# sisl/NeRFSafetyValidation

Hardware: AMD Instinct MI355X
Metric: rendered_samples_per_sec (higher is better)
Workload: dtype f16; 1 GPU; Stonehenge 800x800 synthetic, hashgrid L=16 F=2 T=2^19 + ffmlp(64,2)/(64,3), fp16, occupancy-grid ray marching (run_cuda eval path, BASELINE configs[1]); rays_per_frame=640000, bound=2, cascade=2, frames_in_flight=3, fused_reference_rounding=True, parallelism=single GPU, rccl_ranks=1

## Files before the change

### nerfsafetyvalidation_amd/csrc/fused_net.hpp

```cpp
#pragma once
#include <hip/hip_fp16.h>
#include <math.h>

#include "ngp_common.hpp"

namespace ngp {

typedef _Float16 half8 __attribute__((ext_vector_type(8)));
typedef _Float16 half2v __attribute__((ext_vector_type(2)));
typedef _Float16 half4 __attribute__((ext_vector_type(4)));
typedef float f32x4 __attribute__((ext_vector_type(4)));

struct LevelTab {
    float scale[16];
    uint32_t offset[16], size[16];
    uint32_t a1[16], a2[16];
    uint32_t mask[16];
    uint32_t flags[16];
    uint32_t cell_off[16], cell_res[16];
};

struct NetArgs {
    const uint32_t* table;
    const _Float16* packed;
// ... 859 lines not shown
struct DebugState {
    int flags = 0;
    unsigned long long* stamps = nullptr;
    uint32_t* sample_hash = nullptr;
    bool coarse_off() const { return (flags & 2) != 0; }
    bool sort_off() const { return (flags & 4) != 0; }
    bool lin_off() const { return (flags & 8) != 0; }
    bool jump_off() const { return (flags & 1) != 0; }
    bool spec_off() const { return (flags & 256) != 0; }
    bool tile_off() const { return (flags & 8192) != 0; }
    bool pre_verdict_off() const { return (flags & 16384) != 0; }
    bool narrow_items_off() const { return (flags & 32768) != 0; }
    bool prefix_replay_off() const { return (flags & 65536) != 0; }
    bool wave_march_off() const { return (flags & 131072) != 0; }
    bool cell_runs_off() const { return (flags & 262144) != 0; }
    uint32_t spec_safety_x2() const { return ((uint32_t)flags >> 9) & 15u; }
    uint32_t shrink() const { return ((uint32_t)flags >> 4) & 15u; }
};
DebugState debug_snapshot();
float* grad_dump();
bool needs_generic(const GridLevels& lv);
int fill_net(const ngp_model* m, const DebugState& dbg, const _Float16* packed, NetArgs& na, GridLevels& lv);
size_t weights_bytes(const NetArgs& na);
uint32_t resident_blocks(size_t lds);
int net_variant(const NetArgs& na, const GridLevels& lv);
bool bwd_shape_ok(const NetArgs& na);
#define NGP_WITH_NET(variant, ...)                                           \
    switch (variant) {                                                       \
        case 0: { using NET = NetF16<0>; __VA_ARGS__; } break;               \
        case 1: { using NET = NetF16<1>; __VA_ARGS__; } break;               \
// ... 10 lines not shown
```

### nerfsafetyvalidation_amd/csrc/render_fused.hip

```cpp
#include <hip/hip_fp16.h>
#include <math.h>
#include <string.h>

#include <atomic>

#include "fused_net.hpp"
#include "occupancy.hpp"

namespace ngp {

constexpr int kWaves = 8;
constexpr int kThreads = kWaves * 64;
constexpr int kWavesPerSimd = 4;
constexpr int kCh = 2;
constexpr int kSlots = 64 * kCh;
constexpr size_t kLinMaxBytes = 4u << 20;
constexpr int kLookahead = 4;
constexpr int kRing = 8;

struct Ctl {
    uint32_t n_alive, n_step, step, done;
    uint32_t iters, last_n_alive, last_n_step, pad;
    unsigned long long samples_marched, samples_slots;
    uint32_t spec, rollbacks, backoff, rsv;
// ... 14 lines not shown
    const float *rays_o, *rays_d, *fars;
    float* rays_t;
    float *weights_sum, *depth, *image;
    float *last_sigmas, *last_rgbs;
    float pad_sigma, pad_r, pad_g, pad_b;
    float4* dump_rec;
    uint32_t* dump_iter;
    const int32_t* alive_in;
    int32_t* staging;
    uint32_t* chunk_count;
    uint32_t sort_slow;
    Ctl* ctl;
    QueueHeads* heads;
    unsigned long long* stat_shards;
    uint32_t* death_shards;
    float4* backup;
    const uint8_t* bitfield;
    uint32_t cascade, grid_size, max_steps, perturb;
    float dt_gamma;
    Pcg32 rng;
    OccupancyLin occ;
    uint32_t block_jump;
    uint32_t* sample_hash;
    unsigned long long* stamps;
    float2* march_samples;
    uint8_t* march_counts;
    uint32_t wave_slots;
    uint32_t n_rays;
    uint32_t pre_verdict;
    uint32_t wave_march_max;
// ... 31 lines not shown
    uint16_t list[kSlots];
    float od[64][6];
};

__device__ __forceinline__ void dump_row(const RenderArgs& ra, uint32_t entry, int32_t ray, uint32_t n_step, uint32_t k, float sg, float r,
                                         float g, float b) {
    if (ra.dump_rec) {
        ra.dump_rec[(size_t)ray * 8 + k] = make_float4(sg, r, g, b);
    } else {
        const size_t row = (size_t)entry * n_step + k;
        ra.last_sigmas[row] = sg;
        ra.last_rgbs[row * 3] = r; ra.last_rgbs[row * 3 + 1] = g; ra.last_rgbs[row * 3 + 2] = b;
    }
}

__device__ __forceinline__ void march_ahead_wave(const RenderArgs& ra, float bound, const Ctl& ctl, const uint32_t* coarse) {
    const uint32_t lane = threadIdx.x & 63u;
    const uint32_t entry = blockIdx.x * 4u + (threadIdx.x >> 6);
    if (entry >= ctl.n_alive) return;
    const uint32_t n_step = ctl.n_step, spec = ctl.spec;
    const int32_t ray = ra.alive_in[entry];
    Dda dda;
    const float t_c = ra.rays_t[ray], far = ra.fars[ray];
    float t_march = dda.start(ra.rays_o + (size_t)ray * 3, ra.rays_d + (size_t)ray * 3, ra.bitfield, bound, 0.0f, ra.max_steps, ra.cascade,
                              ra.grid_size, &ra.occ, ra.block_jump != 0, t_c, ra.perturb, ra.rng, entry);
    float last_m = t_march, geo_tc = t_c;
    uint32_t emitted = 0, rounds = 0;
    float2* out = ra.march_samples + ((size_t)(entry >> 6) * n_step) * 64 + (entry & 63u);
    while (t_march < far && emitted < n_step) {
        rounds++;
        const LatticeWindow w = probe_window(dda, t_march, far, lane, coarse);
        const uint32_t room = spec ? spec - emitted % spec : n_step - emitted;
        unsigned long long emit = 0ull;
        uint32_t cur = 0, cnt = 0;
        float t_next = t_march;
        for (int guard = 0; guard < 64; guard++) {
// ... 19 lines not shown
    }
    if (lane != 0) return;
    if (ra.stamps) {
        atomicAdd(ra.stamps + 4, (unsigned long long)rounds);
        atomicAdd(ra.stamps + 5, (unsigned long long)rounds * 64ull);
        atomicAdd(ra.stamps + 6, 1ull);
        atomicMax(ra.stamps + 7, (unsigned long long)rounds);
    }
    if (spec && ra.pre_verdict && emitted < n_step)
        atomicAdd(ra.death_shards + (size_t)kDeathShards * kSpecK + (blockIdx.x % kDeathShards) * kSpecK + emitted / spec, 1u);
    bool slow = false;
    if (ra.sort_slow && emitted == n_step) slow = geo_tc < far && dda.coarse_empty_at_lin(geo_tc, coarse);
    ra.march_counts[entry] = (uint8_t)(emitted | (slow ? 128u : 0u));
}

template <bool LIN>
__global__ void __launch_bounds__(256) k_march_ahead(RenderArgs ra, float bound) {
    const Ctl ctl = *ra.ctl;
    if (ctl.done) return;
    const uint32_t n_alive = ctl.n_alive, n_step = ctl.n_step, spec = ctl.spec;
    const bool by_wave = LIN && n_alive <= ra.wave_march_max;
    if (blockIdx.x * (by_wave ? 4u : 256u) >= n_alive) return;
    __shared__ uint32_t coarse_lds[kCoarseMaxBytes / 4];
    stage_coarse(ra.occ, coarse_lds, blockDim.x);
    __syncthreads();
    const uint32_t* coarse = ra.occ.coarse_words ? coarse_lds : nullptr;
    if (LIN && by_wave) {
        march_ahead_wave(ra, bound, ctl, coarse);
        return;
    }
    const uint32_t entry = blockIdx.x * blockDim.x + threadIdx.x;
    if (entry >= n_alive) return;
    const int32_t ray = ra.alive_in[entry];
    Dda dda;
    const float t_c = ra.rays_t[ray], far = ra.fars[ray];
    float t_march = dda.start(ra.rays_o + (size_t)ray * 3, ra.rays_d + (size_t)ray * 3, ra.bitfield, bound, ra.dt_gamma, ra.max_steps, ra.cascade,
                              ra.grid_size, LIN ? &ra.occ : nullptr, ra.block_jump != 0, t_c, ra.perturb, ra.rng, entry);
    float last_m = t_march;
    float geo_tc = t_c;
    uint32_t emitted = 0;
    float2* out = ra.march_samples + ((size_t)(entry >> 6) * n_step) * 64 + (entry & 63u);
    float x, y, z, dt;
    uint32_t probes = 0, probes_coarse_empty = 0, probes_fine_empty = 0;
    const bool run_cells = LIN && dda.const_dt && ra.cell_runs != 0;
    float occ_until = 0.0f;
    while (t_march < far && emitted < n_step) {
        probes++;
        const bool diag_ce = LIN && ra.stamps && dda.coarse_empty_at_lin(t_march, coarse);
// ... 43 lines not shown
        uint32_t* ex = ra.death_shards + (size_t)kDeathShards * kSpecK + (blockIdx.x % kDeathShards) * kSpecK;
        for (uint32_t j = 0; j < K; j++) {
            const unsigned long long b = __ballot(jd == j);
            if (leader && b) atomicAdd(&ex[j], (uint32_t)__popcll(b));
        }
    }
    bool slow = false;
    if (ra.sort_slow && emitted == n_step) slow = geo_tc < far && (LIN ? dda.coarse_empty_at_lin(geo_tc, coarse) : dda.coarse_empty_at(geo_tc, coarse));
    ra.march_counts[entry] = (uint8_t)(emitted | (slow ? 128u : 0u));
}

template <int MODE, bool HACC = false>
__global__ void __launch_bounds__(kThreads, kWavesPerSimd) k_render_iter(NetArgs na, GridLevels lv, RenderArgs ra) {
    Ctl ctl = *ra.ctl;
    if (ctl.done) return;
    const uint32_t n_step_marched = ctl.n_step;
    extern __shared__ __attribute__((aligned(16))) char smem[];
    if (ctl.spec) {
        uint32_t* exhausted = reinterpret_cast<uint32_t*>(smem);
        if (threadIdx.x < kSpecK) {
            uint32_t d = 0;
            for (int sh = 0; sh < kDeathShards; sh++) d += ra.death_shards[(size_t)kDeathShards * kSpecK + sh * kSpecK + threadIdx.x];
            exhausted[threadIdx.x] = d;
        }
        __syncthreads();
        truncate_launch(ctl, exhausted, ra.n_rays);
        __syncthreads();
    }
    const uint32_t n_alive = ctl.n_alive, n_step = ctl.n_step;
    const uint32_t spec = ctl.spec;
// ... 240 lines not shown
        wave_total += wave_samples;
        if (ra.dump_iter && active) ra.dump_iter[ray] = ctl.iters;
        if (ra.last_sigmas && !ra.dump_rec && !spec && chunk == n_chunks - 1) {
            for (uint32_t i = lane; i < 128; i += 64) {
                const size_t row = (size_t)n_alive * n_step + i;
                ra.last_sigmas[row] = ra.pad_sigma;
                ra.last_rgbs[row * 3] = ra.pad_r; ra.last_rgbs[row * 3 + 1] = ra.pad_g; ra.last_rgbs[row * 3 + 2] = ra.pad_b;
            }
        }
        NGP_STAMP(3)
    }
#undef NGP_STAMP
    if (lane == 0 && wave_total) atomicAdd(&ra.stat_shards[(blockIdx.x * kWaves + wid) % kStatShards], wave_total);
}

__device__ __forceinline__ void publish_status(unsigned long long* host_slot, const Ctl& n, uint32_t seq, unsigned long long* fin = nullptr,
                                               uint32_t call_tag = 0) {
    if (!host_slot) return;
    if (n.done && fin) {
        const unsigned long long tag = (unsigned long long)(0x8000u | (call_tag & 0x7FFFu)) << 48;
        __hip_atomic_store(fin + 0, tag | (n.samples_marched & 0xFFFFFFFFFFFFull), __ATOMIC_RELAXED, __HIP_MEMORY_SCOPE_SYSTEM);
        __hip_atomic_store(fin + 1, tag | (n.samples_slots & 0xFFFFFFFFFFFFull), __ATOMIC_RELAXED, __HIP_MEMORY_SCOPE_SYSTEM);
        __hip_atomic_store(fin + 2, tag | ((unsigned long long)(n.iters & 0xFFFFFFu) << 24) | (n.rollbacks & 0xFFFFFFu), __ATOMIC_RELAXED,
                           __HIP_MEMORY_SCOPE_SYSTEM);
        __hip_atomic_store(fin + 3, tag | ((unsigned long long)n.last_n_alive << 8) | (n.last_n_step & 0xFFu), __ATOMIC_RELAXED,
                           __HIP_MEMORY_SCOPE_SYSTEM);
    }
    const unsigned long long w = ((unsigned long long)seq << 32) | ((unsigned long long)(n.done ? 1u : 0u) << 31) | (n.n_alive & 0x7FFFFFFFu);
    __hip_atomic_store(host_slot, w, __ATOMIC_RELAXED, __HIP_MEMORY_SCOPE_SYSTEM);
}

__global__ void __launch_bounds__(256) k_render_compact(const Ctl* __restrict__ cur, Ctl* __restrict__ nxt, const int32_t* __restrict__ staging,
                                                         const uint32_t* __restrict__ chunk_count, int32_t* __restrict__ alive_out, uint32_t N,
                                                         uint32_t max_steps, const unsigned long long* __restrict__ stat_shards,
                                                         QueueHeads* __restrict__ nxt_heads, unsigned long long* __restrict__ host_slot, uint32_t seq,
                                                         const uint32_t* __restrict__ death_shards, uint32_t spec_allowed, const int32_t* __restrict__ alive_in,
                                                         const float4* __restrict__ backup, float* __restrict__ rays_t, float* __restrict__ weights_sum,
                                                         float* __restrict__ depth, float* __restrict__ image, uint32_t* __restrict__ sample_hash,
                                                         unsigned long long* stat_shards_rw, uint32_t* __restrict__ death_next, uint32_t wave_slots,
                                                         uint32_t cap_mid_max, uint32_t cap_hi, unsigned long long* __restrict__ fin_host, uint32_t call_tag) {
    __shared__ uint32_t red[3][4];
    __shared__ uint32_t off_f[9], off_s[9];
    Ctl c = *cur;
    if (c.done) {
        if (blockIdx.x == 0 && threadIdx.x == 0) {
            *nxt = c;
            publish_status(host_slot, c, seq, fin_host, call_tag);
        }
        return;
    }
    const uint32_t W = item_width(c.n_alive, wave_slots);
    const uint32_t n_chunks = (c.n_alive + W - 1) / W;
    const uint32_t n_blocks = (n_chunks + 7) / 8;
    const uint32_t g = blockIdx.x;
    if (g >= n_blocks) return;
    const uint32_t first = g * 8;
    __shared__ uint32_t deaths[kSpecK], exhausted[kSpecK];
    __shared__ uint32_t verdict_bad, verdict_keep;
    if (threadIdx.x < kSpecK) {
        uint32_t d = 0, x = 0;
        if (c.spec)
            for (int sh = 0; sh < kDeathShards; sh++) {
                d += death_shards[sh * kSpecK + threadIdx.x];
                x += death_shards[(size_t)kDeathShards * kSpecK + sh * kSpecK + threadIdx.x];
            }
        deaths[threadIdx.x] = d;
        exhausted[threadIdx.x] = x;
    }
    __syncthreads();
    truncate_launch(c, exhausted, N);
    if (threadIdx.x == 0) {
        uint32_t bad = 0, keep = 0;
        if (c.spec) {
            const uint32_t q = c.spec, K = c.n_step / q;
            uint32_t alive = c.n_alive;
            keep = K;
            for (uint32_t j = 0; j < K; j++) {
                if (alive == 0) break;
                const uint32_t want_q = N / alive;
                if (j > 0 && (want_q < 1 ? 1u : (want_q > 8 ? 8u : want_q)) != q) { bad = 1; keep = j; break; }
                alive -= deaths[j];
                if ((spec_allowed & 2u) && alive == 0) { bad = 1; keep = j; break; }
            }
        }
        verdict_bad = bad;
        verdict_keep = keep;
    }
    __syncthreads();
    if (verdict_bad) {
        for (uint32_t e = first * W + threadIdx.x; e < (first + 8) * W && e < c.n_alive; e += 256) {
            const int32_t ray = alive_in[e];
            const float4 a = backup[(size_t)ray * 2], b = backup[(size_t)ray * 2 + 1];
            rays_t[ray] = a.x; weights_sum[ray] = a.y; depth[ray] = a.z;
            if (sample_hash) sample_hash[ray] = __float_as_uint(a.w);
            image[(size_t)ray * 3] = b.x; image[(size_t)ray * 3 + 1] = b.y; image[(size_t)ray * 3 + 2] = b.z;
            alive_out[e] = ray;
        }
        if (g == n_blocks - 1 && threadIdx.x == 0) {
            Ctl n = c;
            n.rollbacks = c.rollbacks + 1;
            if (verdict_keep >= 2 && !(spec_allowed & 4u)) {
                n.spec = c.spec;
                n.n_step = verdict_keep * c.spec;
                n.backoff = 0;
                for (uint32_t i = 0; i < kDeathWords; i++) death_next[i] = 0;
            } else {
                n.spec = 0;
                const uint32_t ns = c.n_alive ? N / c.n_alive : 8;
                n.n_step = ns < 1 ? 1 : (ns > 8 ? 8 : ns);
                n.backoff = 2;
            }
            for (int i = 0; i < kStatShards; i++) stat_shards_rw[i] = 0ull;
            *nxt = n;
            for (int i = 0; i < 8; i++) nxt_heads->head[i][0] = 0;
            publish_status(host_slot, n, seq, fin_host, call_tag);
        }
        return;
    }
    uint32_t pf = 0, ps = 0, tf = 0;
    for (uint32_t j = threadIdx.x; j < n_chunks; j += 256) {
        const uint32_t v = chunk_count[j];
        tf += v >> 16;
        if (j < first) { pf += v & 0xffffu; ps += v >> 16; }
    }
#pragma unroll
    for (int off = 32; off > 0; off >>= 1) {
        pf += __shfl_down(pf, off, 64);
        ps += __shfl_down(ps, off, 64);
        tf += __shfl_down(tf, off, 64);
    }
    if ((threadIdx.x & 63) == 0) { red[0][threadIdx.x >> 6] = pf; red[1][threadIdx.x >> 6] = ps; red[2][threadIdx.x >> 6] = tf; }
    if (threadIdx.x == 0) {
        uint32_t af = 0, as = 0;
        for (uint32_t i = 0; i < 8; i++) {
            const uint32_t v = (first + i < n_chunks) ? chunk_count[first + i] : 0;
            off_f[i] = af; off_s[i] = as;
            af += v & 0xffffu; as += v >> 16;
        }
        off_f[8] = af; off_s[8] = as;
    }
    __syncthreads();
    const uint32_t prefix_f = red[0][0] + red[0][1] + red[0][2] + red[0][3];
    const uint32_t prefix_s = red[1][0] + red[1][1] + red[1][2] + red[1][3];
    const uint32_t total_s = red[2][0] + red[2][1] + red[2][2] + red[2][3];
    const uint32_t lane = threadIdx.x & 63, w = threadIdx.x >> 6;
#pragma unroll
    for (uint32_t h = 0; h < 2; h++) {
        const uint32_t ci = w * 2 + h;
        const uint32_t nf = off_f[ci + 1] - off_f[ci], ns = off_s[ci + 1] - off_s[ci];
        if (lane < ns) alive_out[prefix_s + off_s[ci] + lane] = staging[(size_t)(first + ci) * W + W - 1 - lane];
        if (lane < nf) alive_out[total_s + prefix_f + off_f[ci] + lane] = staging[(size_t)(first + ci) * W + lane];
    }
    unsigned long long marched = threadIdx.x < (uint32_t)kStatShards ? stat_shards_rw[threadIdx.x] : 0ull;
#pragma unroll
    for (int off = 32; off > 0; off >>= 1) marched += __shfl_down(marched, off, 64);
    if (g == n_blocks - 1 && threadIdx.x == 0) {
        Ctl n = c;
        n.samples_marched = c.samples_marched + marched;
        for (int i = 0; i < kStatShards; i++) stat_shards_rw[i] = 0ull;
        n.n_alive = total_s + prefix_f + off_f[8];
        uint32_t recent = c.n_alive - n.n_alive;
        if (!c.spec) {
            n.last_n_alive = c.n_alive;
            n.last_n_step = c.n_step;
            n.iters = c.iters + 1;
            n.samples_slots = c.samples_slots + (unsigned long long)c.n_alive * c.n_step;
            n.step = c.step + c.n_step;
        } else {
            const uint32_t q = c.spec, K = c.n_step / q;
            uint32_t alive = c.n_alive, d_last = 0, d_prev = 0;
            unsigned long long slots = c.samples_slots;
            uint32_t it = 0;
            for (uint32_t j = 0; j < K; j++) {
                if (alive == 0) break;
                slots += (unsigned long long)alive * q;
                it++;
                n.last_n_alive = alive;
                n.last_n_step = q;
                alive -= deaths[j];
                d_prev = d_last;
                d_last = deaths[j];
            }
            recent = d_last > d_prev ? d_last : d_prev;
            n.iters = c.iters + it;
            n.samples_slots = slots;
            n.step = c.step + it * q;
        }
        uint32_t ns = n.n_alive ? N / n.n_alive : 8;
        n.n_step = ns < 1 ? 1 : (ns > 8 ? 8 : ns);
        n.done = (n.n_alive == 0 || n.step >= max_steps) ? 1 : 0;
        n.spec = 0;
        if (n.backoff) n.backoff--;
        else if (spec_allowed && !n.done && n.n_step <= kSpecMaxQ && (n.n_step == 8 || n.n_alive > N / (n.n_step + 1))) {
            const uint32_t q = n.n_step;
            const bool own_last = (spec_allowed & 2u) != 0;
            uint32_t room = (max_steps - n.step) / q;
            if (own_last && room) room--;
            const uint32_t headroom = n.n_alive - (q == 8 ? 0u : N / (q + 1)) - 1;
            uint32_t sq = 0;
            while ((unsigned long long)(sq + 1) * (sq + 1) <= recent) sq++;
            const unsigned long long rate = (unsigned long long)recent + 4ull * sq + 16ull;
            const uint32_t safety_x2 = (spec_allowed >> 8) ? (spec_allowed >> 8) : kSpecSafetyX2;
            uint32_t K = (uint32_t)((unsigned long long)headroom * 2u / (safety_x2 * rate));
            const uint32_t cap_mid = 8u * q < cap_mid_max ? 8u * q : cap_mid_max;
            const uint32_t cap_samples = q == 1 ? 8u : (q <= 4 ? cap_mid : cap_hi);
            const uint32_t capK = cap_samples / q < kSpecK ? cap_samples / q : kSpecK;
            K = (q == 8 && !own_last) ? capK : (K < capK ? K : capK);
            K = K < room ? K : room;
            if (K >= 2) { n.spec = q; n.n_step = K * q; }
        }
        if (n.spec)
            for (uint32_t i = 0; i < kDeathWords; i++) death_next[i] = 0;
        *nxt = n;
        for (int i = 0; i < 8; i++) nxt_heads->head[i][0] = 0;
        publish_status(host_slot, n, seq, fin_host, call_tag);
    }
}

__global__ void __launch_bounds__(256) k_render_init(uint32_t N, const float* __restrict__ nears, float* __restrict__ rays_t,
                                                      int32_t* __restrict__ alive, float* __restrict__ weights_sum, float* __restrict__ depth,
                                                      float* __restrict__ image, Ctl* __restrict__ ctl, uint32_t max_steps,
                                                      uint32_t* __restrict__ sample_hash, unsigned long long* __restrict__ stat_shards,
                                                      QueueHeads* __restrict__ heads, uint32_t* __restrict__ death_shards, uint32_t spec_allowed,
                                                      uint32_t tile_w) {
    const uint32_t n = blockIdx.x * 256 + threadIdx.x;
    if (n < (uint32_t)kStatShards) stat_shards[n] = 0ull;
    if (n < 2u * kDeathWords) death_shards[n] = 0;
    if (n < 16) heads[n >> 3].head[n & 7][0] = 0;
    if (n < N) {
        if (sample_hash) sample_hash[n] = 2166136261u;
// ... 299 lines not shown
    uint32_t known = 0;
    uint32_t launches = 2;
    bool done = false;
    while (!done) {
        const uint32_t cur = launched & 1;
        const uint32_t chunks = items_bound(ub, ra.wave_slots);
        static const uint32_t pct_env = getenv("NGP_ITER_BLOCKS_PCT") ? (uint32_t)atoi(getenv("NGP_ITER_BLOCKS_PCT")) : 0u;
        const uint32_t blocks_pct = pct_env ? pct_env : (g_active_renders.load(std::memory_order_relaxed) > 1 ? 62u : 100u);
        const uint32_t max_blocks = (uint32_t)ctx->num_cu * blocks_per_cu * blocks_pct / 100u;
        const uint32_t want_blocks = div_up(chunks, kWaves);
        const uint32_t blocks = want_blocks < max_blocks ? want_blocks : max_blocks;
        ra.alive_in = ctx->alive[cur];
        ra.ctl = ctx->ctl + cur;
        ra.heads = ctx->heads + cur;
        ra.death_shards = ctx->death_shards + (size_t)cur * kDeathWords;
        {
            ProfScope pm("k_march_ahead", s, 0);
            const uint32_t by_wave = div_up(ub < ra.wave_march_max ? ub : ra.wave_march_max, 4);
            const uint32_t by_lane = div_up(ub ? ub : 1, 256);
            if (lin) k_march_ahead<true><<<by_lane > by_wave ? by_lane : by_wave, 256, 0, s>>>(ra, na.bound);
            else k_march_ahead<false><<<div_up(ub ? ub : 1, 256), 256, 0, s>>>(ra, na.bound);
        }
        {
            ProfScope pk("k_render_iter", s, 0);
            iter_kernel<<<blocks, kThreads, lds, s>>>(na, lv, ra);
        }
        k_render_compact<<<div_up(chunks, 8), 256, 0, s>>>(ctx->ctl + cur, ctx->ctl + (cur ^ 1), ctx->staging, ctx->chunk_count,
                                                           ctx->alive[cur ^ 1], N, max_steps, ctx->stat_shards, ctx->heads + (cur ^ 1),
                                                           ctx->status_dev + launched % kRing, ctx->seq_base + launched + 1,
                                                           ctx->death_shards + (size_t)cur * kDeathWords, spec_allowed, ctx->alive[cur],
                                                           ctx->backup, ctx->rays_t, weights_sum, depth, image, dbg.sample_hash, ctx->stat_shards,
                                                           ctx->death_shards + (size_t)(cur ^ 1) * kDeathWords, ra.wave_slots, cap_mid_max, cap_hi, ctx->fin_dev, call_tag);
        launched++;
        launches += 3;
        while (known < launched) {
            static const uint32_t lookahead = getenv("NGP_LOOKAHEAD") ? (uint32_t)atoi(getenv("NGP_LOOKAHEAD")) : (uint32_t)kLookahead;
            const bool must_wait = launched - known >= lookahead;
            volatile unsigned long long* slot = ctx->status + known % kRing;
            const uint32_t want_seq = ctx->seq_base + known + 1;
            unsigned long long w = *slot;
            if ((uint32_t)(w >> 32) != want_seq) {
                if (!must_wait) break;
                uint32_t spins = 0;
                while ((uint32_t)((w = *slot) >> 32) != want_seq) {
                    if ((++spins & 0xFFFFFu) == 0) {
                        const hipError_t q = hipStreamQuery(s);
                        if (q != hipSuccess && q != hipErrorNotReady) {
                            set_error("render_rays: %s", hipGetErrorString(q));
                            return NGP_ELAUNCH;
                        }
                        if (q == hipSuccess && (uint32_t)(*slot >> 32) != want_seq) {
// ... 6 lines not shown
            }
            known++;
            ub = (uint32_t)w & 0x7FFFFFFFu;
            static const bool trace_sched = getenv("NGP_TRACE_SCHEDULE") != nullptr;
            if (trace_sched) fprintf(stderr, "[ngp] call %u launch %u: n_alive %u%s\n", call_tag, known, ub, ((w >> 31) & 1ull) ? " done" : "");
            if ((w >> 31) & 1ull) { done = true; break; }
        }
        if (launched > 2u * max_steps + 16u) {
            set_error("render_rays: iteration bound exceeded");
            return NGP_ELAUNCH;
        }
    }
    ctx->seq_base += launched;
    if (ra.dump_rec) {
        const uint32_t nb = div_up(N, 256);
        const Ctl* fin_state = ctx->ctl + (launched & 1);
        k_dump_count<<<nb, 256, 0, s>>>(ctx->dump_iter, N, fin_state, ctx->chunk_count);
        k_dump_scan<<<1, 1024, 0, s>>>(ctx->chunk_count, nb);
        k_dump_gather<<<nb, 256, 0, s>>>(ctx->dump_iter, ctx->dump_rec, N, fin_state, ctx->chunk_count,
                                         last_sigmas, last_rgbs, ra.pad_sigma, ra.pad_r, ra.pad_g, ra.pad_b);
    }
    rc = check_launch("render_rays");
    if (rc) return rc;
    bool have_fin = false;
    Ctl fin = {};
    if (stats_host && !sync) {
        volatile unsigned long long* f = ctx->fin;
        unsigned long long w[4] = {0, 0, 0, 0};
        for (uint32_t spin = 0; spin < 200000u && !have_fin; spin++) {
            bool all = true;
            for (int i = 0; i < 4; i++) {
// ... 5 lines not shown
        }
        if (have_fin) {
            fin.samples_marched = w[0] & 0xFFFFFFFFFFFFull;
            fin.samples_slots = w[1] & 0xFFFFFFFFFFFFull;
            fin.iters = (uint32_t)((w[2] >> 24) & 0xFFFFFFu);
            fin.rollbacks = (uint32_t)(w[2] & 0xFFFFFFu);
            fin.last_n_alive = (uint32_t)((w[3] >> 8) & 0xFFFFFFFFu);
            fin.last_n_step = (uint32_t)(w[3] & 0xFFu);
        }
    }
    if ((stats_host && !have_fin) || sync) {
        if (hipStreamSynchronize(s) != hipSuccess) {
            set_error("render_rays: %s", hipGetErrorString(hipGetLastError()));
            return NGP_ELAUNCH;
        }
        if (hipMemcpy(&fin, ctx->ctl + (launched & 1), sizeof(Ctl), hipMemcpyDeviceToHost) != hipSuccess) {
            set_error("render_rays: %s", hipGetErrorString(hipGetLastError()));
            return NGP_ELAUNCH;
        }
        have_fin = true;
    }
    if (have_fin) {
        if (stats_host) {
            stats_host->samples_marched = fin.samples_marched;
            stats_host->samples_slots = fin.samples_slots;
            stats_host->iterations = fin.iters;
            stats_host->rays = N;
            stats_host->last_n_alive = fin.last_n_alive;
            stats_host->last_n_step = fin.last_n_step;
            stats_host->launches = launches;
            stats_host->replayed = fin.rollbacks;
// ... 17 lines not shown
```

Baseline: 7.704 billion samples/s.

## Fuse compaction and control-state update into the next march kernel

The per-iteration compaction kernel is removed as a separate launch. Each march block now recomputes the launch verdict and next control state, and gathers its own slice of surviving rays directly from chunk counts and staging before marching. This cuts one kernel launch per iteration and the round trip through the alive list, but every block redundantly reads the death shards and chunk-count prefix. The host scheduling loop is adjusted because the status for an iteration is now published one launch later.

Result: slower. 7.561 billion samples/s (-1.9%).

```diff
diff --git a/nerfsafetyvalidation_amd/csrc/fused_net.hpp b/nerfsafetyvalidation_amd/csrc/fused_net.hpp
--- a/nerfsafetyvalidation_amd/csrc/fused_net.hpp
+++ b/nerfsafetyvalidation_amd/csrc/fused_net.hpp
@@ -897,6 +897,7 @@
     bool prefix_replay_off() const { return (flags & 65536) != 0; }
     bool wave_march_off() const { return (flags & 131072) != 0; }
     bool cell_runs_off() const { return (flags & 262144) != 0; }
+    bool fused_stitch_off() const { return (flags & 524288) != 0; }
     uint32_t spec_safety_x2() const { return ((uint32_t)flags >> 9) & 15u; }
     uint32_t shrink() const { return ((uint32_t)flags >> 4) & 15u; }
 };
diff --git a/nerfsafetyvalidation_amd/csrc/render_fused.hip b/nerfsafetyvalidation_amd/csrc/render_fused.hip
--- a/nerfsafetyvalidation_amd/csrc/render_fused.hip
+++ b/nerfsafetyvalidation_amd/csrc/render_fused.hip
@@ -52,6 +52,7 @@
     QueueHeads* heads;
     unsigned long long* stat_shards;
     uint32_t* death_shards;
+    uint32_t* death_next;
     float4* backup;
     const uint8_t* bitfield;
     uint32_t cascade, grid_size, max_steps, perturb;
@@ -113,12 +114,285 @@
     }
 }
 
-__device__ __forceinline__ void march_ahead_wave(const RenderArgs& ra, float bound, const Ctl& ctl, const uint32_t* coarse) {
+__device__ __forceinline__ void publish_status(unsigned long long* host_slot, const Ctl& n, uint32_t seq, unsigned long long* fin = nullptr,
+                                               uint32_t call_tag = 0) {
+    if (!host_slot) return;
+    if (n.done && fin) {
+        const unsigned long long tag = (unsigned long long)(0x8000u | (call_tag & 0x7FFFu)) << 48;
+        __hip_atomic_store(fin + 0, tag | (n.samples_marched & 0xFFFFFFFFFFFFull), __ATOMIC_RELAXED, __HIP_MEMORY_SCOPE_SYSTEM);
+        __hip_atomic_store(fin + 1, tag | (n.samples_slots & 0xFFFFFFFFFFFFull), __ATOMIC_RELAXED, __HIP_MEMORY_SCOPE_SYSTEM);
+        __hip_atomic_store(fin + 2, tag | ((unsigned long long)(n.iters & 0xFFFFFFu) << 24) | (n.rollbacks & 0xFFFFFFu), __ATOMIC_RELAXED,
+                           __HIP_MEMORY_SCOPE_SYSTEM);
+        __hip_atomic_store(fin + 3, tag | ((unsigned long long)n.last_n_alive << 8) | (n.last_n_step & 0xFFu), __ATOMIC_RELAXED,
+                           __HIP_MEMORY_SCOPE_SYSTEM);
+    }
+    const unsigned long long w = ((unsigned long long)seq << 32) | ((unsigned long long)(n.done ? 1u : 0u) << 31) | (n.n_alive & 0x7FFFFFFFu);
+    __hip_atomic_store(host_slot, w, __ATOMIC_RELAXED, __HIP_MEMORY_SCOPE_SYSTEM);
+}
+
+__device__ __forceinline__ void load_launch_counts(const Ctl& c, const uint32_t* __restrict__ death_shards, uint32_t* deaths, uint32_t* exhausted) {
+    if (threadIdx.x < kSpecK) {
+        uint32_t d = 0, x = 0;
+        if (c.spec)
+            for (int sh = 0; sh < kDeathShards; sh++) {
+                d += death_shards[sh * kSpecK + threadIdx.x];
+                x += death_shards[(size_t)kDeathShards * kSpecK + sh * kSpecK + threadIdx.x];
+            }
+        deaths[threadIdx.x] = d;
+        exhausted[threadIdx.x] = x;
+    }
+}
+__device__ __forceinline__ bool launch_verdict(const Ctl& c, const uint32_t* deaths, uint32_t N, uint32_t spec_allowed, uint32_t& keep) {
+    keep = 0;
+    if (!c.spec) return false;
+    const uint32_t q = c.spec, K = c.n_step / q;
+    uint32_t alive = c.n_alive;
+    keep = K;
+    for (uint32_t j = 0; j < K; j++) {
+        if (alive == 0) break;
+        const uint32_t want_q = N / alive;
+        if (j > 0 && (want_q < 1 ? 1u : (want_q > 8 ? 8u : want_q)) != q) { keep = j; return true; }
+        alive -= deaths[j];
+        if ((spec_allowed & 2u) && alive == 0) { keep = j; return true; }
+    }
+    return false;
+}
+__device__ __forceinline__ Ctl rollback_ctl(const Ctl& c, uint32_t keep, uint32_t N, uint32_t spec_allowed) {
+    Ctl n = c;
+    n.rollbacks = c.rollbacks + 1;
+    if (keep >= 2 && !(spec_allowed & 4u)) {
+        n.spec = c.spec;
+        n.n_step = keep * c.spec;
+        n.backoff = 0;
+    } else {
+        n.spec = 0;
+        const uint32_t ns = c.n_alive ? N / c.n_alive : 8;
+        n.n_step = ns < 1 ? 1 : (ns > 8 ? 8 : ns);
+        n.backoff = 2;
+    }
+    return n;
+}
+__device__ __forceinline__ Ctl next_ctl(const Ctl& c, const uint32_t* deaths, uint32_t n_alive_new, unsigned long long marched, uint32_t N,
+                                        uint32_t max_steps, uint32_t spec_allowed, uint32_t cap_mid_max, uint32_t cap_hi) {
+    Ctl n = c;
+    n.samples_marched = c.samples_marched + marched;
+    n.n_alive = n_alive_new;
+    uint32_t recent = c.n_alive - n.n_alive;
+    if (!c.spec) {
+        n.last_n_alive = c.n_alive;
+        n.last_n_step = c.n_step;
+        n.iters = c.iters + 1;
+        n.samples_slots = c.samples_slots + (unsigned long long)c.n_alive * c.n_step;
+        n.step = c.step + c.n_step;
+    } else {
+        const uint32_t q = c.spec, K = c.n_step / q;
+        uint32_t alive = c.n_alive, d_last = 0, d_prev = 0;
+        unsigned long long slots = c.samples_slots;
+        uint32_t it = 0;
+        for (uint32_t j = 0; j < K; j++) {
+            if (alive == 0) break;
+            slots += (unsigned long long)alive * q;
+            it++;
+            n.last_n_alive = alive;
+            n.last_n_step = q;
+            alive -= deaths[j];
+            d_prev = d_last;
+            d_last = deaths[j];
+        }
+        recent = d_last > d_prev ? d_last : d_prev;
+        n.iters = c.iters + it;
+        n.samples_slots = slots;
+        n.step = c.step + it * q;
+    }
+    uint32_t ns = n.n_alive ? N / n.n_alive : 8;
+    n.n_step = ns < 1 ? 1 : (ns > 8 ? 8 : ns);
+    n.done = (n.n_alive == 0 || n.step >= max_steps) ? 1 : 0;
+    n.spec = 0;
+    if (n.backoff) n.backoff--;
+    else if (spec_allowed && !n.done && n.n_step <= kSpecMaxQ && (n.n_step == 8 || n.n_alive > N / (n.n_step + 1))) {
+        const uint32_t q = n.n_step;
+        const bool own_last = (spec_allowed & 2u) != 0;
+        uint32_t room = (max_steps - n.step) / q;
+        if (own_last && room) room--;
+        const uint32_t headroom = n.n_alive - (q == 8 ? 0u : N / (q + 1)) - 1;
+        uint32_t sq = (uint32_t)sqrtf((float)recent);
+        while ((unsigned long long)sq * sq > recent) sq--;
+        while ((unsigned long long)(sq + 1) * (sq + 1) <= recent) sq++;
+        const unsigned long long rate = (unsigned long long)recent + 4ull * sq + 16ull;
+        const uint32_t safety_x2 = (spec_allowed >> 8) ? (spec_allowed >> 8) : kSpecSafetyX2;
+        uint32_t K = (uint32_t)((unsigned long long)headroom * 2u / (safety_x2 * rate));
+        const uint32_t cap_mid = 8u * q < cap_mid_max ? 8u * q : cap_mid_max;
+        const uint32_t cap_samples = q == 1 ? 8u : (q <= 4 ? cap_mid : cap_hi);
+        const uint32_t capK = cap_samples / q < kSpecK ? cap_samples / q : kSpecK;
+        K = (q == 8 && !own_last) ? capK : (K < capK ? K : capK);
+        K = K < room ? K : room;
+        if (K >= 2) { n.spec = q; n.n_step = K * q; }
+    }
+    return n;
+}
+__device__ __forceinline__ void restore_ray(const RenderArgs& ra, int32_t ray) {
+    const float4 a = ra.backup[(size_t)ray * 2], b = ra.backup[(size_t)ray * 2 + 1];
+    ra.rays_t[ray] = a.x; ra.weights_sum[ray] = a.y; ra.depth[ray] = a.z;
+    if (ra.sample_hash) ra.sample_hash[ray] = __float_as_uint(a.w);
+    ra.image[(size_t)ray * 3] = b.x; ra.image[(size_t)ray * 3 + 1] = b.y; ra.image[(size_t)ray * 3 + 2] = b.z;
+}
+
+struct StitchArgs {
+    const Ctl* prev;
+    const int32_t* alive_prev;
+    int32_t* alive_out;
+    const uint32_t* death_prev;
+    unsigned long long* host_slot;
+    uint32_t seq;
+    uint32_t spec_allowed, cap_mid_max, cap_hi;
+    unsigned long long* fin_host;
+    uint32_t call_tag;
+};
+
+__device__ __forceinline__ bool march_by_wave(const RenderArgs& ra, uint32_t n_alive) {
+    return n_alive <= ra.wave_march_max && (unsigned long long)gridDim.x * 4ull >= n_alive;
+}
+
+template <bool LIN>
+__device__ __forceinline__ bool stitch_block(const RenderArgs& ra, const StitchArgs& st, Ctl& ctl, bool& by_wave, uint32_t* slot) {
+    __shared__ uint32_t deaths[kSpecK], exhausted[kSpecK];
+    __shared__ uint32_t sub_f[64], sub_s[64];
+    __shared__ Ctl next_state;
+    const uint32_t tid = threadIdx.x, lane = tid & 63u, w = tid >> 6;
+    const uint32_t N = ra.n_rays;
+    Ctl c = *st.prev;
+    if (c.done) {
+        if (blockIdx.x == 0 && tid == 0) {
+            *ra.ctl = c;
+            publish_status(st.host_slot, c, st.seq, st.fin_host, st.call_tag);
+        }
+        return false;
+    }
+    {
+        const uint32_t wave_cap = !LIN ? 0u : (c.n_alive < ra.wave_march_max ? c.n_alive : ra.wave_march_max);
+        if (blockIdx.x * 256u >= c.n_alive && blockIdx.x * 4u >= wave_cap) return false;
+    }
+    load_launch_counts(c, st.death_prev, deaths, exhausted);
+    const uint32_t W = item_width(c.n_alive, ra.wave_slots);
+    const uint32_t n_chunks = (c.n_alive + W - 1) / W;
+    const uint32_t n_groups = (n_chunks + 63u) / 64u, per_sub = (n_groups + 63u) / 64u;
+    {
+        const uint32_t r = tid >> 2, first = r * per_sub * 64u, vecs = per_sub * 16u;
+        uint32_t f = 0, s = 0;
+        for (uint32_t i = tid & 3u; i < vecs; i += 4u) {
+            const uint32_t j = first + 4u * i;
+            if (j >= n_chunks) break;
+            const uint4 v = *reinterpret_cast<const uint4*>(ra.chunk_count + j);
+            f += v.x & 0xffffu; s += v.x >> 16;
+            if (j + 1u < n_chunks) { f += v.y & 0xffffu; s += v.y >> 16; }
+            if (j + 2u < n_chunks) { f += v.z & 0xffffu; s += v.z >> 16; }
+            if (j + 3u < n_chunks) { f += v.w & 0xffffu; s += v.w >> 16; }
+        }
+        f += __shfl_xor(f, 1, 64); s += __shfl_xor(s, 1, 64);
+        f += __shfl_xor(f, 2, 64); s += __shfl_xor(s, 2, 64);
+        if ((tid & 3u) == 0) { sub_f[r] = f; sub_s[r] = s; }
+    }
+    __syncthreads();
+    truncate_launch(c, exhausted, N);
+    uint32_t keep = 0;
+    if (launch_verdict(c, deaths, N, st.spec_allowed, keep)) {
+        const Ctl n = rollback_ctl(c, keep, N, st.spec_allowed);
+        if (blockIdx.x == 0 && tid == 0) {
+            for (int i = 0; i < kStatShards; i++) ra.stat_shards[i] = 0ull;
+            *ra.ctl = n;
+            for (int i = 0; i < 8; i++) ra.heads->head[i][0] = 0;
+            publish_status(st.host_slot, n, st.seq, st.fin_host, st.call_tag);
+        }
+        by_wave = LIN && march_by_wave(ra, n.n_alive);
+        const uint32_t E = by_wave ? 4u : 256u, B = blockIdx.x * E;
+        if (B >= n.n_alive) return false;
+        if (tid < E && B + tid < n.n_alive) {
+            const int32_t ray = st.alive_prev[B + tid];
+            restore_ray(ra, ray);
+            st.alive_out[B + tid] = ray;
+            slot[tid] = (uint32_t)ray;
+        }
+        ctl = n;
+        return true;
+    }
+    unsigned long long marched = 0ull;
+    if (blockIdx.x == 0 && w == 0) {
+        marched = ra.stat_shards[lane];
+#pragma unroll
+        for (int off = 32; off > 0; off >>= 1) marched += __shfl_down(marched, off, 64);
+    }
+    const uint32_t tf = sub_f[lane], ts = sub_s[lane];
+    uint32_t inf = tf, ins = ts;
+#pragma unroll
+    for (int off = 1; off < 64; off <<= 1) {
+        const uint32_t of = __shfl_up(inf, off, 64), os = __shfl_up(ins, off, 64);
+        if (lane >= (uint32_t)off) { inf += of; ins += os; }
+    }
+    const uint32_t total_f = __shfl(inf, 63, 64), total_s = __shfl(ins, 63, 64);
+    const uint32_t exf = inf - tf, exs = ins - ts;
+    const uint32_t n_new = total_s + total_f;
+    if (tid == 0) {
+        const Ctl n = next_ctl(c, deaths, n_new, marched, N, ra.max_steps, st.spec_allowed, st.cap_mid_max, st.cap_hi);
+        if (blockIdx.x == 0) {
+            for (int i = 0; i < kStatShards; i++) ra.stat_shards[i] = 0ull;
+            *ra.ctl = n;
+            for (int i = 0; i < 8; i++) ra.heads->head[i][0] = 0;
+            publish_status(st.host_slot, n, st.seq, st.fin_host, st.call_tag);
+        }
+        next_state = n;
+    }
+    __syncthreads();
+    ctl = next_state;
+    if (ctl.done) return false;
+    by_wave = LIN && march_by_wave(ra, n_new);
+    const uint32_t E = by_wave ? 4u : 256u, B = blockIdx.x * E;
+    if (B >= n_new) return false;
+    const uint32_t hi = B + E < n_new ? B + E : n_new;
+    const uint32_t s_lo = B, s_hi = hi < total_s ? hi : total_s;
+    const uint32_t f_lo = (B > total_s ? B : total_s) - total_s, f_hi = hi > total_s ? hi - total_s : 0u;
+    const bool reach = (s_lo < s_hi && exs < s_hi && exs + ts > s_lo) || (f_lo < f_hi && exf < f_hi && exf + tf > f_lo);
+    unsigned long long need = __ballot(reach);
+    for (uint32_t k = 0; need; k++) {
+        const uint32_t r = (uint32_t)__builtin_ctzll(need);
+        need &= need - 1ull;
+        if ((k & 3u) != w) continue;
+        uint32_t bf = __shfl(exf, (int)r, 64), bs = __shfl(exs, (int)r, 64);
+        const uint32_t g0 = r * per_sub, g1 = g0 + per_sub < n_groups ? g0 + per_sub : n_groups;
+        for (uint32_t g = g0; g < g1; g++) {
+            if ((s_lo >= s_hi || bs >= s_hi) && (f_lo >= f_hi || bf >= f_hi)) break;
+            const uint32_t j = g * 64u + lane;
+            const uint32_t v = j < n_chunks ? ra.chunk_count[j] : 0u;
+            uint32_t inc = v;
+#pragma unroll
+            for (int off = 1; off < 64; off <<= 1) {
+                const uint32_t o = __shfl_up(inc, off, 64);
+                if (lane >= (uint32_t)off) inc += o;
+            }
+            const uint32_t gt = __shfl(inc, 63, 64);
+            const uint32_t nf = v & 0xffffu, ns = v >> 16;
+            const uint32_t ef = bf + (inc & 0xffffu) - nf, es = bs + (inc >> 16) - ns;
+            const uint32_t base = j * W;
+            for (uint32_t o = es > s_lo ? es : s_lo; o < es + ns && o < s_hi; o++) slot[o - B] = base + W - 1u - (o - es);
+            for (uint32_t o = ef > f_lo ? ef : f_lo; o < ef + nf && o < f_hi; o++) slot[o + total_s - B] = base + (o - ef);
+            bf += gt & 0xffffu; bs += gt >> 16;
+        }
+    }
+    __syncthreads();
+    if (tid < E && B + tid < n_new) {
+        const uint32_t src = slot[tid], last = n_chunks * W - 1u;
+        const int32_t ray = ra.staging[src < last ? src : last];
+        st.alive_out[B + tid] = ray;
+        slot[tid] = (uint32_t)ray;
+    }
+    return true;
+}
+
+__device__ __forceinline__ void march_ahead_wave(const RenderArgs& ra, float bound, const Ctl& ctl, const uint32_t* coarse, const uint32_t* stitched) {
     const uint32_t lane = threadIdx.x & 63u;
     const uint32_t entry = blockIdx.x * 4u + (threadIdx.x >> 6);
     if (entry >= ctl.n_alive) return;
     const uint32_t n_step = ctl.n_step, spec = ctl.spec;
-    const int32_t ray = ra.alive_in[entry];
+    const int32_t ray = stitched ? (int32_t)stitched[threadIdx.x >> 6] : ra.alive_in[entry];
     Dda dda;
     const float t_c = ra.rays_t[ray], far = ra.fars[ray];
     float t_march = dda.start(ra.rays_o + (size_t)ray * 3, ra.rays_d + (size_t)ray * 3, ra.bitfield, bound, 0.0f, ra.max_steps, ra.cascade,
@@ -168,24 +442,32 @@
     ra.march_counts[entry] = (uint8_t)(emitted | (slow ? 128u : 0u));
 }
 
-template <bool LIN>
-__global__ void __launch_bounds__(256) k_march_ahead(RenderArgs ra, float bound) {
-    const Ctl ctl = *ra.ctl;
-    if (ctl.done) return;
+template <bool LIN, bool STITCH>
+__global__ void __launch_bounds__(256) k_march_ahead(RenderArgs ra, float bound, StitchArgs st) {
+    __shared__ uint32_t coarse_lds[kCoarseMaxBytes / 4];
+    __shared__ uint32_t stitched[256];
+    Ctl ctl;
+    bool by_wave = false;
+    if (STITCH) {
+        stage_coarse(ra.occ, coarse_lds, blockDim.x);
+        if (!stitch_block<LIN>(ra, st, ctl, by_wave, stitched)) return;
+    } else {
+        ctl = *ra.ctl;
+        if (ctl.done) return;
+        by_wave = LIN && march_by_wave(ra, ctl.n_alive);
+        if (blockIdx.x * (by_wave ? 4u : 256u) >= ctl.n_alive) return;
+    }
     const uint32_t n_alive = ctl.n_alive, n_step = ctl.n_step, spec = ctl.spec;
-    const bool by_wave = LIN && n_alive <= ra.wave_march_max;
-    if (blockIdx.x * (by_wave ? 4u : 256u) >= n_alive) return;
-    __shared__ uint32_t coarse_lds[kCoarseMaxBytes / 4];
-    stage_coarse(ra.occ, coarse_lds, blockDim.x);
+    if (!STITCH) stage_coarse(ra.occ, coarse_lds, blockDim.x);
     __syncthreads();
     const uint32_t* coarse = ra.occ.coarse_words ? coarse_lds : nullptr;
     if (LIN && by_wave) {
-        march_ahead_wave(ra, bound, ctl, coarse);
+        march_ahead_wave(ra, bound, ctl, coarse, STITCH ? stitched : nullptr);
         return;
     }
     const uint32_t entry = blockIdx.x * blockDim.x + threadIdx.x;
     if (entry >= n_alive) return;
-    const int32_t ray = ra.alive_in[entry];
+    const int32_t ray = STITCH ? (int32_t)stitched[threadIdx.x] : ra.alive_in[entry];
     Dda dda;
     const float t_c = ra.rays_t[ray], far = ra.fars[ray];
     float t_march = dda.start(ra.rays_o + (size_t)ray * 3, ra.rays_d + (size_t)ray * 3, ra.bitfield, bound, ra.dt_gamma, ra.max_steps, ra.cascade,
@@ -259,6 +541,8 @@
 __global__ void __launch_bounds__(kThreads, kWavesPerSimd) k_render_iter(NetArgs na, GridLevels lv, RenderArgs ra) {
     Ctl ctl = *ra.ctl;
     if (ctl.done) return;
+    if (blockIdx.x == 0)
+        for (uint32_t i = threadIdx.x; i < kDeathWords; i += kThreads) ra.death_next[i] = 0;
     const uint32_t n_step_marched = ctl.n_step;
     extern __shared__ __attribute__((aligned(16))) char smem[];
     if (ctl.spec) {
@@ -529,112 +813,48 @@
     if (lane == 0 && wave_total) atomicAdd(&ra.stat_shards[(blockIdx.x * kWaves + wid) % kStatShards], wave_total);
 }
 
-__device__ __forceinline__ void publish_status(unsigned long long* host_slot, const Ctl& n, uint32_t seq, unsigned long long* fin = nullptr,
-                                               uint32_t call_tag = 0) {
-    if (!host_slot) return;
-    if (n.done && fin) {
-        const unsigned long long tag = (unsigned long long)(0x8000u | (call_tag & 0x7FFFu)) << 48;
-        __hip_atomic_store(fin + 0, tag | (n.samples_marched & 0xFFFFFFFFFFFFull), __ATOMIC_RELAXED, __HIP_MEMORY_SCOPE_SYSTEM);
-        __hip_atomic_store(fin + 1, tag | (n.samples_slots & 0xFFFFFFFFFFFFull), __ATOMIC_RELAXED, __HIP_MEMORY_SCOPE_SYSTEM);
-        __hip_atomic_store(fin + 2, tag | ((unsigned long long)(n.iters & 0xFFFFFFu) << 24) | (n.rollbacks & 0xFFFFFFu), __ATOMIC_RELAXED,
-                           __HIP_MEMORY_SCOPE_SYSTEM);
-        __hip_atomic_store(fin + 3, tag | ((unsigned long long)n.last_n_alive << 8) | (n.last_n_step & 0xFFu), __ATOMIC_RELAXED,
-                           __HIP_MEMORY_SCOPE_SYSTEM);
-    }
-    const unsigned long long w = ((unsigned long long)seq << 32) | ((unsigned long long)(n.done ? 1u : 0u) << 31) | (n.n_alive & 0x7FFFFFFFu);
-    __hip_atomic_store(host_slot, w, __ATOMIC_RELAXED, __HIP_MEMORY_SCOPE_SYSTEM);
-}
-
-__global__ void __launch_bounds__(256) k_render_compact(const Ctl* __restrict__ cur, Ctl* __restrict__ nxt, const int32_t* __restrict__ staging,
-                                                         const uint32_t* __restrict__ chunk_count, int32_t* __restrict__ alive_out, uint32_t N,
-                                                         uint32_t max_steps, const unsigned long long* __restrict__ stat_shards,
-                                                         QueueHeads* __restrict__ nxt_heads, unsigned long long* __restrict__ host_slot, uint32_t seq,
-                                                         const uint32_t* __restrict__ death_shards, uint32_t spec_allowed, const int32_t* __restrict__ alive_in,
-                                                         const float4* __restrict__ backup, float* __restrict__ rays_t, float* __restrict__ weights_sum,
-                                                         float* __restrict__ depth, float* __restrict__ image, uint32_t* __restrict__ sample_hash,
-                                                         unsigned long long* stat_shards_rw, uint32_t* __restrict__ death_next, uint32_t wave_slots,
-                                                         uint32_t cap_mid_max, uint32_t cap_hi, unsigned long long* __restrict__ fin_host, uint32_t call_tag) {
+
+__global__ void __launch_bounds__(256) k_render_compact(RenderArgs ra, StitchArgs st) {
     __shared__ uint32_t red[3][4];
     __shared__ uint32_t off_f[9], off_s[9];
-    Ctl c = *cur;
+    const uint32_t N = ra.n_rays;
+    Ctl c = *st.prev;
     if (c.done) {
         if (blockIdx.x == 0 && threadIdx.x == 0) {
-            *nxt = c;
-            publish_status(host_slot, c, seq, fin_host, call_tag);
+            *ra.ctl = c;
+            publish_status(st.host_slot, c, st.seq, st.fin_host, st.call_tag);
         }
         return;
     }
-    const uint32_t W = item_width(c.n_alive, wave_slots);
+    const uint32_t W = item_width(c.n_alive, ra.wave_slots);
     const uint32_t n_chunks = (c.n_alive + W - 1) / W;
     const uint32_t n_blocks = (n_chunks + 7) / 8;
     const uint32_t g = blockIdx.x;
     if (g >= n_blocks) return;
     const uint32_t first = g * 8;
     __shared__ uint32_t deaths[kSpecK], exhausted[kSpecK];
-    __shared__ uint32_t verdict_bad, verdict_keep;
-    if (threadIdx.x < kSpecK) {
-        uint32_t d = 0, x = 0;
-        if (c.spec)
-            for (int sh = 0; sh < kDeathShards; sh++) {
-                d += death_shards[sh * kSpecK + threadIdx.x];
-                x += death_shards[(size_t)kDeathShards * kSpecK + sh * kSpecK + threadIdx.x];
-            }
-        deaths[threadIdx.x] = d;
-        exhausted[threadIdx.x] = x;
-    }
+    load_launch_counts(c, st.death_prev, deaths, exhausted);
     __syncthreads();
     truncate_launch(c, exhausted, N);
-    if (threadIdx.x == 0) {
-        uint32_t bad = 0, keep = 0;
-        if (c.spec) {
-            const uint32_t q = c.spec, K = c.n_step / q;
-            uint32_t alive = c.n_alive;
-            keep = K;
-            for (uint32_t j = 0; j < K; j++) {
-                if (alive == 0) break;
-                const uint32_t want_q = N / alive;
-                if (j > 0 && (want_q < 1 ? 1u : (want_q > 8 ? 8u : want_q)) != q) { bad = 1; keep = j; break; }
-                alive -= deaths[j];
-                if ((spec_allowed & 2u) && alive == 0) { bad = 1; keep = j; break; }
-            }
-        }
-        verdict_bad = bad;
-        verdict_keep = keep;
-    }
-    __syncthreads();
-    if (verdict_bad) {
+    uint32_t keep = 0;
+    if (launch_verdict(c, deaths, N, st.spec_allowed, keep)) {
         for (uint32_t e = first * W + threadIdx.x; e < (first + 8) * W && e < c.n_alive; e += 256) {
-            const int32_t ray = alive_in[e];
-            const float4 a = backup[(size_t)ray * 2], b = backup[(size_t)ray * 2 + 1];
-            rays_t[ray] = a.x; weights_sum[ray] = a.y; depth[ray] = a.z;
-            if (sample_hash) sample_hash[ray] = __float_as_uint(a.w);
-            image[(size_t)ray * 3] = b.x; image[(size_t)ray * 3 + 1] = b.y; image[(size_t)ray * 3 + 2] = b.z;
-            alive_out[e] = ray;
+            const int32_t ray = st.alive_prev[e];
+            restore_ray(ra, ray);
+            st.alive_out[e] = ray;
         }
         if (g == n_blocks - 1 && threadIdx.x == 0) {
-            Ctl n = c;
-            n.rollbacks = c.rollbacks + 1;
-            if (verdict_keep >= 2 && !(spec_allowed & 4u)) {
-                n.spec = c.spec;
-                n.n_step = verdict_keep * c.spec;
-                n.backoff = 0;
-                for (uint32_t i = 0; i < kDeathWords; i++) death_next[i] = 0;
-            } else {
-                n.spec = 0;
-                const uint32_t ns = c.n_alive ? N / c.n_alive : 8;
-                n.n_step = ns < 1 ? 1 : (ns > 8 ? 8 : ns);
-                n.backoff = 2;
-            }
-            for (int i = 0; i < kStatShards; i++) stat_shards_rw[i] = 0ull;
-            *nxt = n;
-            for (int i = 0; i < 8; i++) nxt_heads->head[i][0] = 0;
-            publish_status(host_slot, n, seq, fin_host, call_tag);
+            const Ctl n = rollback_ctl(c, keep, N, st.spec_allowed);
+            for (int i = 0; i < kStatShards; i++) ra.stat_shards[i] = 0ull;
+            *ra.ctl = n;
+            for (int i = 0; i < 8; i++) ra.heads->head[i][0] = 0;
+            publish_status(st.host_slot, n, st.seq, st.fin_host, st.call_tag);
         }
         return;
     }
     uint32_t pf = 0, ps = 0, tf = 0;
     for (uint32_t j = threadIdx.x; j < n_chunks; j += 256) {
-        const uint32_t v = chunk_count[j];
+        const uint32_t v = ra.chunk_count[j];
         tf += v >> 16;
         if (j < first) { pf += v & 0xffffu; ps += v >> 16; }
     }
@@ -648,7 +868,7 @@
     if (threadIdx.x == 0) {
         uint32_t af = 0, as = 0;
         for (uint32_t i = 0; i < 8; i++) {
-            const uint32_t v = (first + i < n_chunks) ? chunk_count[first + i] : 0;
+            const uint32_t v = (first + i < n_chunks) ? ra.chunk_count[first + i] : 0;
             off_f[i] = af; off_s[i] = as;
             af += v & 0xffffu; as += v >> 16;
         }
@@ -663,72 +883,18 @@
     for (uint32_t h = 0; h < 2; h++) {
         const uint32_t ci = w * 2 + h;
         const uint32_t nf = off_f[ci + 1] - off_f[ci], ns = off_s[ci + 1] - off_s[ci];
-        if (lane < ns) alive_out[prefix_s + off_s[ci] + lane] = staging[(size_t)(first + ci) * W + W - 1 - lane];
-        if (lane < nf) alive_out[total_s + prefix_f + off_f[ci] + lane] = staging[(size_t)(first + ci) * W + lane];
-    }
-    unsigned long long marched = threadIdx.x < (uint32_t)kStatShards ? stat_shards_rw[threadIdx.x] : 0ull;
+        if (lane < ns) st.alive_out[prefix_s + off_s[ci] + lane] = ra.staging[(size_t)(first + ci) * W + W - 1 - lane];
+        if (lane < nf) st.alive_out[total_s + prefix_f + off_f[ci] + lane] = ra.staging[(size_t)(first + ci) * W + lane];
+    }
+    unsigned long long marched = threadIdx.x < (uint32_t)kStatShards ? ra.stat_shards[threadIdx.x] : 0ull;
 #pragma unroll
     for (int off = 32; off > 0; off >>= 1) marched += __shfl_down(marched, off, 64);
     if (g == n_blocks - 1 && threadIdx.x == 0) {
-        Ctl n = c;
-        n.samples_marched = c.samples_marched + marched;
-        for (int i = 0; i < kStatShards; i++) stat_shards_rw[i] = 0ull;
-        n.n_alive = total_s + prefix_f + off_f[8];
-        uint32_t recent = c.n_alive - n.n_alive;
-        if (!c.spec) {
-            n.last_n_alive = c.n_alive;
-            n.last_n_step = c.n_step;
-            n.iters = c.iters + 1;
-            n.samples_slots = c.samples_slots + (unsigned long long)c.n_alive * c.n_step;
-            n.step = c.step + c.n_step;
-        } else {
-            const uint32_t q = c.spec, K = c.n_step / q;
-            uint32_t alive = c.n_alive, d_last = 0, d_prev = 0;
-            unsigned long long slots = c.samples_slots;
-            uint32_t it = 0;
-            for (uint32_t j = 0; j < K; j++) {
-                if (alive == 0) break;
-                slots += (unsigned long long)alive * q;
-                it++;
-                n.last_n_alive = alive;
-                n.last_n_step = q;
-                alive -= deaths[j];
-                d_prev = d_last;
-                d_last = deaths[j];
-            }
-            recent = d_last > d_prev ? d_last : d_prev;
-            n.iters = c.iters + it;
-            n.samples_slots = slots;
-            n.step = c.step + it * q;
-        }
-        uint32_t ns = n.n_alive ? N / n.n_alive : 8;
-        n.n_step = ns < 1 ? 1 : (ns > 8 ? 8 : ns);
-        n.done = (n.n_alive == 0 || n.step >= max_steps) ? 1 : 0;
-        n.spec = 0;
-        if (n.backoff) n.backoff--;
-        else if (spec_allowed && !n.done && n.n_step <= kSpecMaxQ && (n.n_step == 8 || n.n_alive > N / (n.n_step + 1))) {
-            const uint32_t q = n.n_step;
-            const bool own_last = (spec_allowed & 2u) != 0;
-            uint32_t room = (max_steps - n.step) / q;
-            if (own_last && room) room--;
-            const uint32_t headroom = n.n_alive - (q == 8 ? 0u : N / (q + 1)) - 1;
-            uint32_t sq = 0;
-            while ((unsigned long long)(sq + 1) * (sq + 1) <= recent) sq++;
-            const unsigned long long rate = (unsigned long long)recent + 4ull * sq + 16ull;
-            const uint32_t safety_x2 = (spec_allowed >> 8) ? (spec_allowed >> 8) : kSpecSafetyX2;
-            uint32_t K = (uint32_t)((unsigned long long)headroom * 2u / (safety_x2 * rate));
-            const uint32_t cap_mid = 8u * q < cap_mid_max ? 8u * q : cap_mid_max;
-            const uint32_t cap_samples = q == 1 ? 8u : (q <= 4 ? cap_mid : cap_hi);
-            const uint32_t capK = cap_samples / q < kSpecK ? cap_samples / q : kSpecK;
-            K = (q == 8 && !own_last) ? capK : (K < capK ? K : capK);
-            K = K < room ? K : room;
-            if (K >= 2) { n.spec = q; n.n_step = K * q; }
-        }
-        if (n.spec)
-            for (uint32_t i = 0; i < kDeathWords; i++) death_next[i] = 0;
-        *nxt = n;
-        for (int i = 0; i < 8; i++) nxt_heads->head[i][0] = 0;
-        publish_status(host_slot, n, seq, fin_host, call_tag);
+        const Ctl n = next_ctl(c, deaths, total_s + prefix_f + off_f[8], marched, N, ra.max_steps, st.spec_allowed, st.cap_mid_max, st.cap_hi);
+        for (int i = 0; i < kStatShards; i++) ra.stat_shards[i] = 0ull;
+        *ra.ctl = n;
+        for (int i = 0; i < 8; i++) ra.heads->head[i][0] = 0;
+        publish_status(st.host_slot, n, st.seq, st.fin_host, st.call_tag);
     }
 }
 
@@ -1058,27 +1224,43 @@
         ra.ctl = ctx->ctl + cur;
         ra.heads = ctx->heads + cur;
         ra.death_shards = ctx->death_shards + (size_t)cur * kDeathWords;
+        ra.death_next = ctx->death_shards + (size_t)(cur ^ 1) * kDeathWords;
+        StitchArgs st = {};
+        const bool stitch = launched > 0;
+        if (stitch) {
+            st.prev = ctx->ctl + (cur ^ 1); st.alive_prev = ctx->alive[cur ^ 1]; st.alive_out = ctx->alive[cur];
+            st.death_prev = ctx->death_shards + (size_t)(cur ^ 1) * kDeathWords;
+            st.host_slot = ctx->status_dev + (launched - 1) % kRing; st.seq = ctx->seq_base + launched;
+            st.spec_allowed = spec_allowed; st.cap_mid_max = cap_mid_max; st.cap_hi = cap_hi;
+            st.fin_host = ctx->fin_dev; st.call_tag = call_tag;
+        }
+        const bool fused = stitch && !dbg.fused_stitch_off();
+        if (stitch && !fused) {
+            k_render_compact<<<div_up(chunks, 8), 256, 0, s>>>(ra, st);
+            launches++;
+        }
         {
             ProfScope pm("k_march_ahead", s, 0);
-            const uint32_t by_wave = div_up(ub < ra.wave_march_max ? ub : ra.wave_march_max, 4);
+            const uint32_t by_wave = ub <= 2u * ra.wave_march_max ? div_up(ub < ra.wave_march_max ? ub : ra.wave_march_max, 4) : 0u;
             const uint32_t by_lane = div_up(ub ? ub : 1, 256);
-            if (lin) k_march_ahead<true><<<by_lane > by_wave ? by_lane : by_wave, 256, 0, s>>>(ra, na.bound);
-            else k_march_ahead<false><<<div_up(ub ? ub : 1, 256), 256, 0, s>>>(ra, na.bound);
+            const uint32_t grid = lin && by_wave > by_lane ? by_wave : by_lane;
+            if (lin) {
+                if (fused) k_march_ahead<true, true><<<grid, 256, 0, s>>>(ra, na.bound, st);
+                else k_march_ahead<true, false><<<grid, 256, 0, s>>>(ra, na.bound, st);
+            } else {
+                if (fused) k_march_ahead<false, true><<<grid, 256, 0, s>>>(ra, na.bound, st);
+                else k_march_ahead<false, false><<<grid, 256, 0, s>>>(ra, na.bound, st);
+            }
         }
         {
             ProfScope pk("k_render_iter", s, 0);
             iter_kernel<<<blocks, kThreads, lds, s>>>(na, lv, ra);
         }
-        k_render_compact<<<div_up(chunks, 8), 256, 0, s>>>(ctx->ctl + cur, ctx->ctl + (cur ^ 1), ctx->staging, ctx->chunk_count,
-                                                           ctx->alive[cur ^ 1], N, max_steps, ctx->stat_shards, ctx->heads + (cur ^ 1),
-                                                           ctx->status_dev + launched % kRing, ctx->seq_base + launched + 1,
-                                                           ctx->death_shards + (size_t)cur * kDeathWords, spec_allowed, ctx->alive[cur],
-                                                           ctx->backup, ctx->rays_t, weights_sum, depth, image, dbg.sample_hash, ctx->stat_shards,
-                                                           ctx->death_shards + (size_t)(cur ^ 1) * kDeathWords, ra.wave_slots, cap_mid_max, cap_hi, ctx->fin_dev, call_tag);
         launched++;
-        launches += 3;
-        while (known < launched) {
-            static const uint32_t lookahead = getenv("NGP_LOOKAHEAD") ? (uint32_t)atoi(getenv("NGP_LOOKAHEAD")) : (uint32_t)kLookahead;
+        launches += 2;
+        while (known + 1 < launched) {
+            static const uint32_t lookahead_env = getenv("NGP_LOOKAHEAD") ? (uint32_t)atoi(getenv("NGP_LOOKAHEAD")) : (uint32_t)kLookahead;
+            static const uint32_t lookahead = lookahead_env < 2u ? 2u : lookahead_env;
             const bool must_wait = launched - known >= lookahead;
             volatile unsigned long long* slot = ctx->status + known % kRing;
             const uint32_t want_seq = ctx->seq_base + known + 1;
@@ -1115,7 +1297,7 @@
     ctx->seq_base += launched;
     if (ra.dump_rec) {
         const uint32_t nb = div_up(N, 256);
-        const Ctl* fin_state = ctx->ctl + (launched & 1);
+        const Ctl* fin_state = ctx->ctl + ((launched - 1) & 1);
         k_dump_count<<<nb, 256, 0, s>>>(ctx->dump_iter, N, fin_state, ctx->chunk_count);
         k_dump_scan<<<1, 1024, 0, s>>>(ctx->chunk_count, nb);
         k_dump_gather<<<nb, 256, 0, s>>>(ctx->dump_iter, ctx->dump_rec, N, fin_state, ctx->chunk_count,
@@ -1151,7 +1333,7 @@
             set_error("render_rays: %s", hipGetErrorString(hipGetLastError()));
             return NGP_ELAUNCH;
         }
-        if (hipMemcpy(&fin, ctx->ctl + (launched & 1), sizeof(Ctl), hipMemcpyDeviceToHost) != hipSuccess) {
+        if (hipMemcpy(&fin, ctx->ctl + ((launched - 1) & 1), sizeof(Ctl), hipMemcpyDeviceToHost) != hipSuccess) {
             set_error("render_rays: %s", hipGetErrorString(hipGetLastError()));
             return NGP_ELAUNCH;
         }
```
